# catid/longhair

Hardware: AMD Instinct MI355X
Metric: GB/s of input data encoded+decoded, device-resident, per GPU and whole node (higher is better)
Workload: dtype u8

## Files before the change

longhair_amd/csrc/codec.cpp:

```cpp
#include <hip/hip_runtime.h>

#include <algorithm>
#include <atomic>
#include <cstdio>
#include <cstdlib>
#include <cstring>
#include <map>
#include <memory>
#include <mutex>
#include <stdexcept>
#include <thread>
#include <string>
#include <vector>

#include "../../include/cauchy_256.h"
#include "../../include/cauchy_256_batch.h"
#include "field.hpp"
#include "jit.hpp"
#include "host_codec.hpp"
#include "kernels.hpp"

namespace lh {

enum { kOk = 0, kInvalid = -1, kNoDevice = -2, kHipError = -3 };
// ... 444 lines not shown
                        stride * (cfg.spw ? cfg.spw : 1) < (1ll << 31);
    const JitKernels *jk = nullptr;
    std::string err;
    if (jit_ok) {
        bool hard = false;
        jk = jit_lookup(d, cfg, allow_compile, &err, &hard);
        if (hard) return fail(kHipError, err);
    }
    JitConfig fcfg;
    if (!jk && k > 1 && m > 1 && !cfg.family && jit_family_config_for(k, m, bytes, &fcfg, true) &&
        stride * fcfg.spw < (1ll << 31)) {
        std::string ferr;
        bool fhard = false;
        if (const JitKernels *fk = jit_lookup(d, fcfg, allow_compile, &ferr, &fhard)) {
            if (fk->decode_fused) {
                jk = fk;
                cfg = fcfg;
            }
        }
    }
    const bool generic = (k > 1 && m > 1) && !jk;
    if (jk && jk->decode_fused && std::getenv("LONGHAIR_AMD_NO_FUSED_PLAN") == nullptr) {
        const uint8_t *zero = nullptr;
        if (int rc = zero_page(d, (size_t)bytes, &zero, st)) return rc;
        hipFunction_t fn = jk->decode_fused;
        long long s1 = stride;
        const uint8_t *gexp = d->gf_exp;
        const int16_t *glog = d->gf_log;
        int n = stripes, bb = bytes;
        void *args[] = {(void *)&d_blocks, &s1, (void *)&d_rows, (void *)&d_status, (void *)&zero,
                        (void *)&gexp, (void *)&glog, &n, &bb};
        const long long waves = cfg.spw ? (stripes + cfg.spw - 1) / cfg.spw : (long long)stripes * cfg.wps;
        const int wpb = cfg.family ? 4 : cfg.dec_wpb;
        LH_HIP(hipModuleLaunchKernel(fn, (unsigned)((waves + wpb - 1) / wpb), 1, 1, 64u * (unsigned)wpb, 1, 1,
                                     jk->dyn_lds, st, args, nullptr));
        note_launch(cfg.family ? "lh_jit_decode_fused(family)" : "lh_jit_decode_fused");
        return kOk;
    }
    JitConfig wcfg;
    const JitKernels *wk = nullptr;
    if (generic && jit_win_config_for(k, m, bytes, &wcfg, true)) {
        bool hard = false;
        wk = jit_lookup(d, wcfg, allow_compile, &err, &hard);
        if (hard) return fail(kHipError, err);
        if (wk && !wk->decode_wide) wk = nullptr;
    }
    const int sub = bytes / 8, jnch = (sub + 3) / 4;
    const bool jump = generic && !wk && sub >= 4 && !(sub % 4 != 0 && jnch > 1 && (jnch - 1) % 64 == 0);
    const size_t work_bytes = (generic && !wk && !jump) ? (size_t)stripes * e_max * bytes : 0;
    Workspace *w = nullptr;
    if (int rc = run_planner(d, st, k, m, e_max, stripes, d_rows, d_status, work_bytes, generic && !wk, &w)) return rc;
    if (k <= 1) return kOk;

    if (m == 1) {
        XorArgs a{};
        a.in = d_blocks;
        a.in_stride = stride;
        a.out = d_blocks;
        a.out_stride = stride;
        a.plan = w->plan.ptr;
        a.plan_stride = plan_stride;
        a.k = k;
        a.m = m;
        a.e_max = e_max;
        a.n_in = k;
        a.n_rep = 1;
        a.bytes = bytes;
        a.stripes = stripes;
// ... 1040 lines not shown
```

longhair_amd/csrc/jit.cpp:

```cpp
#include "jit.hpp"

#include <hip/hiprtc.h>
#include <dlfcn.h>
#include <sys/stat.h>
#include <unistd.h>
#include <utime.h>

#include <algorithm>
#include <cstdio>
#include <cstdlib>
#include <cstring>
#include <deque>
#include <functional>
#include <sstream>
#include <thread>

#include "field.hpp"

extern "C" const char lh_jit_source[];
extern "C" const char lh_inv_jump_source[];

namespace lh {

namespace {
// ... 67 lines not shown
    cfg->bytes = bytes;
    cfg->sub = sub;
    cfg->W = W;
    cfg->nch = nch2;
    cfg->spw = spw;
    cfg->wps = wps;
    cfg->lds = 0;
    if (W == 8 && nch2 <= 64 && bytes % 16 == 0) {
        bool dpp_ok = true;
        if (sub - 8 * (nch2 - 1) != 8)
            for (int s = 0; s < spw; ++s) dpp_ok = dpp_ok && (s * nch2 + nch2 - 1) % 16 != 0;
        cfg->lds = dpp_ok ? 1 : 0;
        const long long lq = ((long long)spw * bytes + 1023) / 1024;
        if (!decode && 4 * (4 * lq * 1024 + 16) + 4ll * spw * (k + m) * 8 > 80 * 1024) cfg->lds = 0;
    }
    cfg->role = decode ? 2 : 1;
    cfg->plain = decode && !(emax <= 4 && nch2 <= 64 && k <= 64 && std::getenv("LONGHAIR_AMD_NO_FUSED_PLAN") == nullptr);
    cfg->defines.clear();
    if (const char *d = std::getenv("LONGHAIR_AMD_JIT_DEFINES")) cfg->defines = d;
    auto knob = [&](const char *name, int dflt) {
        const size_t at = cfg->defines.find(name);
        return at == std::string::npos ? dflt : std::atoi(cfg->defines.c_str() + at + std::strlen(name));
    };
    const bool dmo = decode && cfg->lds && !cfg->plain && knob("LH_DMO=", 0) == 1;
    cfg->cps = 1;
    if ((!decode || dmo) && cfg->lds) cfg->cps = std::max(1, std::min(5, k / 2));
    cfg->cps = knob("LH_CPS=", cfg->cps);
    if (cfg->cps > 1 && !((!decode || dmo) && cfg->lds && k >= 2 * cfg->cps)) cfg->cps = 1;
    cfg->wgcu = knob("LH_WGCU=", cfg->cps > 1 ? 1 : 0);
    const int wpb = knob("LH_WPB=", 4);
    cfg->enc_wpb = (cfg->cps > 1 && wpb >= 1 && wpb <= 8) ? wpb : 4;
    const int dwpb = knob("LH_DWPB=", 4);
    cfg->dec_wpb = (decode && !cfg->plain && dwpb >= 1 && dwpb <= 8) ? dwpb : 4;
    cfg->family = 0;
    if (allow_family && knob("LH_FAMILY=", 0) && jit_family_config_for(k, m, bytes, cfg, decode)) return true;
    return true;
}

bool jit_family_config_for(int k, int m, int bytes, JitConfig *cfg, bool decode) {
    if (const char *env = std::getenv("LONGHAIR_AMD_PATH")) {
        if (std::string(env) == "generic") return false;
    }
    if (!jit_family_ok(k, m, bytes, decode)) return false;
    if (decode && std::getenv("LONGHAIR_AMD_NO_FUSED_PLAN") != nullptr) return false;
    JitConfig c;
    c.k = k;
    c.m = m;
    c.bytes = bytes;
    c.sub = bytes / 8;
    c.W = 8;
    c.nch = (c.sub + 7) / 8;
    c.spw = 64 / c.nch;
    c.wps = 0;
    c.lds = 1;
    c.role = decode ? 2 : 1;
    c.plain = 0;
    c.family = 1;
    if (const char *d = std::getenv("LONGHAIR_AMD_JIT_DEFINES")) c.defines = d;
    auto knob = [&](const char *name, int dflt) {
        const size_t at = c.defines.find(name);
        return at == std::string::npos ? dflt : std::atoi(c.defines.c_str() + at + std::strlen(name));
    };
    c.cps = std::max(2, std::min(5, k / 2));
    if (knob("LH_LDS=", 1) == 0 || knob("LH_CPS=", c.cps) < 2 || knob("LH_WPB=", 4) != 4) return false;
    c.wgcu = knob("LH_WGCU=", decode ? 0 : 1);
    c.enc_wpb = 4;
    *cfg = c;
    return true;
}

bool jit_ptr_config_for(int k, int m, int bytes, bool decode, JitConfig *cfg) {
    if (!config_impl(k, m, bytes, decode, cfg, false)) return false;
    cfg->cps = 1;
    cfg->enc_wpb = 4;
    if (cfg->defines.find("LH_WGCU=") == std::string::npos) cfg->wgcu = 0;
    if ((long long)(cfg->spw ? cfg->spw : 1) * k > 1024) return false;
    cfg->ptr = 1;
    const long long spw = cfg->spw ? cfg->spw : 1;
    if (decode && 4 * spw * (k + 1) * 8 > 4096) cfg->lds = 0;
    return true;
}

bool jit_win_ptr_config_for(int k, int m, int bytes, JitConfig *cfg, bool decode) {
    if (!jit_win_config_for(k, m, bytes, cfg, decode)) return false;
    cfg->ptr = 1;
    return true;
}

bool jit_win_config_for(int k, int m, int bytes, JitConfig *cfg, bool decode) {
    if (const char *env = std::getenv("LONGHAIR_AMD_PATH")) {
        if (std::string(env) == "generic") return false;
    }
    if (k < 2 || m < 2 || k + m > 256 || bytes % 8 != 0 || bytes <= 0) return false;
    const int sub = bytes / 8, W = 4;
    if (sub % (64 * W) != 0) return false;
    cfg->k = k;
    cfg->m = m;
    cfg->bytes = bytes;
    cfg->sub = sub;
// ... 281 lines not shown
       << "  const int p = (int)(blockIdx.x % lh_cps) * " << 64 * c.W << " + (int)(threadIdx.x & 63) * "
       << c.W << ";\n"
       << "  const unsigned char *b = in + stripe * in_stride + p;\n"
       << "  unsigned char *o = out + stripe * out_stride + p;\n";
    os << "  const unsigned char *sb = in + stripe * in_stride + (int)(blockIdx.x % lh_cps) * " << 64 * c.W
       << ";\n";
    const char *eargs = "(b, o, sb, nullptr, bytes, lh_sub)";
    for (int g = 0; g < NG; ++g) os << "  " << (g ? "else " : "") << "if (g == " << g << ") lh_wg" << g << eargs << ";\n";
    os << "}\n";
    return os.str();
}

std::string jit_source_for(const JitConfig &c) {
    std::ostringstream os;
    if (c.win) {
        std::string tok;
        for (char ch : c.defines + " ") {
            if (ch == ' ' || ch == ',') {
                const size_t eq = tok.find('=');
                if (!tok.empty()) os << "#define " << (eq == std::string::npos ? tok : tok.substr(0, eq) + " " + tok.substr(eq + 1)) << "\n";
                tok.clear();
            } else {
                tok += ch;
            }
        }
        os << win_source_for(c);
        return os.str();
    }
    {
        std::string tok;
        for (char ch : c.defines + " ") {
            if (ch == ' ' || ch == ',') {
                const size_t eq = tok.find('=');
                if (!tok.empty()) os << "#define " << (eq == std::string::npos ? tok : tok.substr(0, eq) + " " + tok.substr(eq + 1)) << "\n";
                tok.clear();
            } else {
                tok += ch;
            }
        }
    }
    if (c.family) {
        os << "#define LH_FAMILY 1\n#define LH_K " << c.k << "\n#define LH_M " << c.m
           << "\n#define LH_BYTES 1024\n#define LH_SUB 128\n#define LH_W 8\n#define LH_NCH 16\n#define LH_SPW 4"
              "\n#define LH_WPS 1\n#ifndef LH_LDS\n#define LH_LDS 1\n#endif\n#ifndef LH_CPS\n#define LH_CPS "
           << c.cps << "\n#endif\n#define LH_ROLE " << c.role << "\n#define LH_DEC_PLAIN 0\n";
    } else {
    os << "#define LH_K " << c.k << "\n#define LH_M " << c.m << "\n#define LH_BYTES " << c.bytes
       << "\n#define LH_SUB " << c.sub << "\n#define LH_W " << c.W << "\n#define LH_NCH " << c.nch
       << "\n#define LH_SPW " << (c.spw ? c.spw : 1) << "\n#define LH_WPS " << (c.wps ? c.wps : 1) << "\n";
    if (c.ptr) os << "#define LH_PTR 1\n#define LH_BUF 0\n";
    if (c.lds) os << "#ifndef LH_LDS\n#define LH_LDS 1\n#endif\n";
    if (c.cps > 1 && !c.ptr) os << "#ifndef LH_CPS\n#define LH_CPS " << c.cps << "\n#endif\n";
    if (c.role) os << "#define LH_ROLE " << c.role << "\n#define LH_DEC_PLAIN " << c.plain << "\n";
    }
    const std::vector<uint8_t> g = generator_matrix(c.k, c.m);
    os << "static constexpr unsigned char LH_BM[" << c.m << "][" << c.k << "][8] = {";
    for (int r = 0; r < c.m; ++r) {
        os << "{";
        for (int x = 0; x < c.k; ++x) {
            const uint64_t bm = bitmatrix(g[(size_t)r * c.k + x]);
            os << "{";
            for (int y = 0; y < 8; ++y) os << (unsigned)((bm >> (8 * y)) & 0xFF) << (y < 7 ? "," : "");
            os << "}" << (x + 1 < c.k ? "," : "");
        }
        os << "}" << (r + 1 < c.m ? "," : "");
    }
    os << "};\n";
// ... 364 lines not shown
```

longhair_amd/csrc/jit.hpp:

```cpp
#pragma once

#include <hip/hip_runtime.h>

#include <condition_variable>
#include <cstdint>
#include <map>
#include <memory>
#include <mutex>
#include <string>
#include <tuple>
#include <vector>

namespace lh {

struct JitConfig {
    int k, m, bytes, sub;
    int W;
    int nch;
    int spw;
    int wps;
    std::string defines;
    int win = 0;
    int rows_per_wave = 8;
    int win_pf = 3;
    int win_lds = 1;
    int win_split = 1;
    int ptr = 0;
    int lds = 0;
    int role = 0;
    int plain = 0;
    int wgcu = 0;
    int cps = 1;
    int family = 0;
    int enc_wpb = 4;
    int dec_wpb = 4;
    int lanes_per_launch_unit() const { return 64; }
};

struct JitKernels {
    hipModule_t module = nullptr;
    hipFunction_t encode = nullptr;
    hipFunction_t decode = nullptr;
    hipFunction_t decode_fused = nullptr;
    hipFunction_t encode_win = nullptr;
    hipFunction_t decode_wide = nullptr;
    unsigned dyn_lds = 0;
    JitConfig cfg{};
};

bool jit_config_for(int k, int m, int bytes, bool decode, JitConfig *cfg);

bool jit_ptr_config_for(int k, int m, int bytes, bool decode, JitConfig *cfg);

bool jit_win_config_for(int k, int m, int bytes, JitConfig *cfg, bool decode = false);
bool jit_win_ptr_config_for(int k, int m, int bytes, JitConfig *cfg, bool decode = false);

long long generator_ones(int k, int m);

bool jit_family_ok(int k, int m, int bytes, bool decode = false);
bool jit_family_config_for(int k, int m, int bytes, JitConfig *cfg, bool decode = false);

enum class JitMode {
    kCached,
    kAsync,
    kBlocking,
};

class JitCache {
// ... 36 lines not shown
```

longhair_amd/csrc/jit_codec.hip:

```cpp

#ifndef LH_K
#define LH_K 4
#define LH_M 2
#define LH_BYTES 64
#define LH_SUB 8
#define LH_W 8
#define LH_NCH 1
#define LH_SPW 64
#define LH_WPS 0
static constexpr unsigned char LH_BM[LH_M][LH_K][8] = {
    {{1, 2, 4, 8, 16, 32, 64, 128}, {1, 2, 4, 8, 16, 32, 64, 128},
     {1, 2, 4, 8, 16, 32, 64, 128}, {1, 2, 4, 8, 16, 32, 64, 128}},
    {{1, 2, 4, 8, 16, 32, 64, 128}, {2, 4, 8, 16, 32, 64, 128, 135},
     {3, 6, 12, 24, 48, 96, 192, 7}, {4, 8, 16, 32, 64, 128, 135, 137}}};
#define LH_G_INIT {{1, 1, 1, 1}, {1, 2, 3, 4}}
#include <hip/hip_runtime.h>
#endif

#define LH_NW ((LH_W + 3) / 4)


struct lh_word {
    unsigned int v[LH_NW];
};
// ... 1383 lines not shown
extern "C" __global__ void __launch_bounds__(256)
lh_jit_decode(unsigned char *__restrict__ blocks, long long stripe_stride,
              const unsigned char *__restrict__ plan, long long plan_stride,
              const unsigned char *__restrict__ zero_page, int stripes) {
    LH_WAVE_LOOP(stripes) { lh_decode_wave(lh_w, blocks, stripe_stride, plan, plan_stride, zero_page, stripes); }
}
#endif

#if LH_EMAX <= 4 && LH_NCH <= 64 && LH_K <= 64
#define LH_FUSED 1
#ifndef LH_DWPB
#define LH_DWPB 4
#endif
static constexpr unsigned char LH_GRAW[LH_M][LH_K] = LH_G_INIT;
#define LH_P4(n) (((n) + 3) / 4 * 4)
#define LH_SR (2 * LH_P4(LH_K) + LH_P4(LH_M))
#define LH_NRW ((LH_K + LH_NCH - 1) / LH_NCH)
#define LH_STRIPE_LANES (LH_NCH >= 64 ? ~0ull : ((1ull << (LH_NCH & 63)) - 1))

struct lh_gct {
    static constexpr int nch = LH_NCH, nrw = LH_NRW, maxrw = LH_NRW;
    static constexpr unsigned long long lanes = LH_STRIPE_LANES;
};

template <class G>
__device__ __forceinline__ void lh_fused_rows(const G &g, const lh_lane &l, int c, const unsigned char *__restrict__ rows,
                                              unsigned int (&rowv)[G::maxrw]) {
    const unsigned char *grow = rows + l.stripe * LH_K;
#pragma unroll
    for (int t = 0; t < G::maxrw; ++t) {
        const int i = c + t * g.nch;
        rowv[t] = (l.active && t < g.nrw && i < LH_K) ? (unsigned int)grow[i] : 0u;
    }
}

__device__ __forceinline__ unsigned int lh_gmul(const unsigned char *gexp, const short *glog, unsigned int a,
                                                unsigned int b) {
    return (a && b) ? gexp[glog[a] + glog[b]] : 0u;
}

struct lh_fused_solve {
    unsigned int rs[LH_EMAX], rr[LH_EMAX], er[LH_EMAX];
    unsigned char *grow;
    const unsigned char *gexp;
    const short *glog;
    const unsigned char *gmat;
    int c;
    __device__ __forceinline__ void operator()(lh_plan_regs &pr) const;
};

template <class G>
__device__ __forceinline__ bool lh_fused_plan(const G &g, const lh_lane &l, int c, int sl, unsigned char *scr,
                                              const unsigned int (&rowv)[G::maxrw],
                                              unsigned char *__restrict__ rows, signed char *__restrict__ status,
                                              lh_fused_solve &sv, lh_plan_regs &pr) {
    unsigned char *lrows = scr;
    unsigned char *lsrc = scr + LH_P4(LH_K);
    unsigned char *lrec = lsrc + LH_P4(LH_K);
    unsigned char *grow = rows + l.stripe * LH_K;
    for (int q = c; q < (LH_P4(LH_K) + LH_P4(LH_M)) / 4; q += g.nch) ((unsigned int *)lsrc)[q] = 0xFFFFFFFFu;
    bool bad = false;
#pragma unroll
    for (int t = 0; t < G::maxrw; ++t) {
        const int i = c + t * g.nch;
        if (t >= g.nrw || i >= LH_K) continue;
        const unsigned int r = rowv[t];
// ... 367 lines not shown
            }
#endif
#pragma unroll
            for (int y = 0; y < 8; ++y) {
                lh_word w = o[y];
                if constexpr (VL != 8) {
                    const lh_word f = lh_funnel<VL>(lh_row_shr1(w.v[0]), lh_row_shr1(w.v[1]), w.v[0], w.v[1]);
                    w.v[0] = last ? f.v[0] : w.v[0];
                    w.v[1] = last ? f.v[1] : w.v[1];
                }
#if LH_DEC_ST_PEND
                if (y == 7) {
                    pend = w;
                    pd = d;
                    continue;
                }
#endif
                lh_store(d + y * sub, w);
                asm volatile("" ::: "memory");
            }
        }
    }
#if LH_DEC_ST_PEND
    if (e > 0) lh_store(pd + 7 * sub, pend);
#endif
}
template <class DST>
__device__ __forceinline__ void lh_fused_out(const lh_word (&v)[LH_M][8], const lh_plan_regs &pr, bool last, DST dst) {
    lh_fused_out_g<LH_VLAST>(v, pr, last, LH_SUB, dst);
}
__device__ __forceinline__ void lh_fused_wave_lds(const lh_lane &l, long long wave, int c, int sl, bool work,
                                                  const unsigned char *scr, unsigned char *__restrict__ blocks,
                                                  long long stripe_stride, int stripes, const lh_fused_solve &sv,
                                                  lh_plan_regs &pr, const unsigned char *zero_page) {
    __shared__ __attribute__((aligned(16))) unsigned char lh_dring[LH_DWPB][LH_LD * LH_LQ * 1024 + LH_LPAD];
    const int lane = threadIdx.x & 63;
    const long long s0 = (long long)__builtin_amdgcn_readfirstlane((int)wave) * LH_SPW;
    if (s0 >= stripes) return;
    const int nst = (int)((stripes - s0) < LH_SPW ? (stripes - s0) : LH_SPW);
    const unsigned long long wm = __ballot(work);
    if (wm == 0) return;
    lh_dldsrc S;
#if LH_PTR
    __shared__ unsigned long long lh_dpt[LH_DWPB][LH_SPW * (LH_K + 1)];
    unsigned long long *prow = lh_dpt[threadIdx.x >> 6];
    __builtin_amdgcn_fence(__ATOMIC_RELEASE, "wavefront");
    __builtin_amdgcn_wave_barrier();
    if (sl < nst) {
        const unsigned long long *t = (const unsigned long long *)(blocks + (s0 + sl) * stripe_stride);
        for (int x = c; x <= LH_K; x += LH_NCH)
            prow[sl * (LH_K + 1) + x] = x < LH_K ? t[x] : (unsigned long long)zero_page;
    }
    __builtin_amdgcn_fence(__ATOMIC_RELEASE, "wavefront");
    __builtin_amdgcn_wave_barrier();
    __builtin_amdgcn_fence(__ATOMIC_ACQUIRE, "wavefront");
    S.pt = prow;
#else
    (void)zero_page;
#if LH_ASM_DMA
    S.rs = lh_rsrc(blocks + s0 * stripe_stride, (unsigned)(nst * stripe_stride));
#else
    S.rs = __builtin_amdgcn_make_buffer_rsrc(blocks + s0 * stripe_stride, 0, (int)(nst * stripe_stride), 0x00020000);
#endif
#endif
    S.scr = scr;
    S.ring = lh_dring[lh_wid<1>()];
#pragma unroll
    for (int q = 0; q < LH_LQ; ++q) {
        int j = 64 * q + lane;
        if (j >= nst * (LH_BYTES / 16)) j = nst * (LH_BYTES / 16) - 1;
        const int js = j / (LH_BYTES / 16);
#if LH_PTR
        S.prow[q] = js * (LH_K + 1);
        S.joff[q] = (j - js * (LH_BYTES / 16)) * 16;
#else
        S.joff[q] = js * (int)stripe_stride + (j - js * (LH_BYTES / 16)) * 16;
#endif
        S.jsc[q] = js * LH_SR | (((wm >> (js * LH_NCH)) & 1ull) ? 0 : (int)0x80000000);
    }
    asm volatile("s_waitcnt lgkmcnt(0)" ::: "memory");
    lh_decode_lds_prologue(S);
    if (work) sv(pr);
    lh_word v[LH_M][8];
#pragma unroll
    for (int r = 0; r < LH_M; ++r)
#pragma unroll
        for (int y = 0; y < 8; ++y)
#pragma unroll
            for (int i = 0; i < LH_NW; ++i) v[r][y].v[i] = 0;
    const int lo = (sl < LH_SPW ? sl : LH_SPW - 1) * LH_BYTES + 8 * c;
    int lo8 = lo + 8;
    asm volatile("" : "+v"(lo8));
    lh_unroll_decode_lds<0>::run(v, S, lo, lo8);
    if (!work) return;
#if LH_PTR
    lh_fused_out(v, pr, l.last, [&](int slot) {
        return (unsigned char *)S.pt[sl * (LH_K + 1) + slot] + (l.last ? LH_SUB - 8 : 8 * c);
    });
#else
    unsigned char *base = blocks + l.stripe * stripe_stride + (l.last ? LH_SUB - 8 : 8 * c);
    lh_fused_out(v, pr, l.last, [&](int slot) { return base + (long long)slot * LH_BYTES; });
#endif
}
#endif

#ifndef LH_DMO
#define LH_DMO 0
#endif
#if LH_DMO && !(LH_LDS && LH_CPS > 1 && !LH_PTR && defined(LH_FUSED))
#undef LH_DMO
#define LH_DMO 0
#endif
#if LH_DMO
#ifndef LH_DMO_AHEAD
// ... 51 lines not shown
        constexpr int S = (B * LH_SUB) % 8;
        if constexpr (S == 0) {
            d[B].v[0] = x[B].x;
            d[B].v[1] = x[B].y;
        } else {
            d[B] = lh_funnel<S>(x[B].x, x[B].y, y[B].x, y[B].y);
        }
        lh_dmo_fn<B + 1>(d, x, y);
    }
}
__device__ __forceinline__ void lh_dmo_col(lh_word (&d)[8], const unsigned char *col, int lo, int lo8) {
    lh_u32x2a x[8], y[8];
    lh_dmo_rd<0>(x, y, col, lo, lo8);
#pragma unroll
    for (int b = 0; b < 8; ++b) {
        asm volatile("" : "+v"(x[b]));
        if ((b * LH_SUB) % 8 != 0) asm volatile("" : "+v"(y[b]));
    }
    lh_dmo_fn<0>(d, x, y);
}
__device__ __forceinline__ void lh_dmo_issue(const lh_u32x4r &rs, const int (&voff)[LH_SQ], int t, unsigned char *ring) {
    const int lane = threadIdx.x & 63;
    const bool lastep = t + 1 == LH_NSTEP;
#pragma unroll
    for (int q = 0; q < LH_SQ; ++q) {
        int v = voff[q];
        if (LH_LASTC < LH_CPS && lastep) v = ((64 * q + lane) % LH_SCH) < LH_LASTC * LH_CCH ? v : (int)0x80000000;
        lh_dma16_bufs<LH_LDS_NT_DEC>(rs, v, t * (LH_CPS * LH_BYTES), ring + q * 1024);
    }
}
__device__ __forceinline__ void lh_fused_wave_dmo(const lh_lane &l, long long wave, int c, int sl, bool work,
                                                  const unsigned char *scr, unsigned char *__restrict__ blocks,
                                                  long long stripe_stride, int stripes, const lh_fused_solve &sv,
                                                  lh_plan_regs &pr) {
    __shared__ __attribute__((aligned(16))) unsigned char lh_mring[LH_DWPB][(1 + LH_DMO_AHEAD) * LH_SSLOT];
    const int lane = threadIdx.x & 63;
    const long long s0 = (long long)__builtin_amdgcn_readfirstlane((int)wave) * LH_SPW;
    if (s0 >= stripes) return;
    const int nst = (int)((stripes - s0) < LH_SPW ? (stripes - s0) : LH_SPW);
    const unsigned long long wm = __ballot(work);
    if (wm == 0) return;
    unsigned char *ring = lh_mring[lh_wid<1>()];
    const lh_u32x4r rs = lh_rsrc(blocks + s0 * stripe_stride, (unsigned)(nst * stripe_stride));
    int voff[LH_SQ];
#pragma unroll
    for (int q = 0; q < LH_SQ; ++q) {
        const int j = 64 * q + lane, js = j / LH_SCH, r = j - js * LH_SCH;
        const bool on = js < nst && ((wm >> (js * LH_NCH)) & 1ull);
        voff[q] = on ? js * (int)stripe_stride + r * 16 : (int)0x80000000;
    }
    asm volatile("s_waitcnt lgkmcnt(0)" ::: "memory");
    lh_dmo_issue(rs, voff, 0, ring);
    if (work) sv(pr);
    lh_word v[LH_M][8];
#pragma unroll
    for (int r = 0; r < LH_M; ++r)
#pragma unroll
        for (int y = 0; y < 8; ++y)
#pragma unroll
            for (int i = 0; i < LH_NW; ++i) v[r][y].v[i] = 0;
    const int sc = sl < LH_SPW ? sl : LH_SPW - 1;
    const int lo = sc * (LH_CPS * LH_BYTES) + 8 * c;
    int lo8 = lo + 8;
    asm volatile("" : "+v"(lo8));
    const unsigned char *lrows = scr + sc * LH_SR;
#pragma unroll 1
    for (int t = 0; t < LH_NSTEP; ++t) {
#if LH_DMO_AHEAD
        unsigned char *cur = ring + (t & 1) * LH_SSLOT;
        if (t + 1 < LH_NSTEP) {
            lh_dmo_issue(rs, voff, t + 1, ring + ((t + 1) & 1) * LH_SSLOT);
            lh_wait_vmcnt<LH_SQ>();
        } else {
            lh_wait_vmcnt<0>();
        }
#else
        unsigned char *cur = ring;
        lh_wait_vmcnt<0>();
#endif
        asm volatile("" ::: "memory");
        const int ncol = t + 1 < LH_NSTEP ? LH_CPS : LH_LASTC;
#pragma unroll 1
        for (int cc = 0; cc < ncol; ++cc) {
            lh_word d[8];
            lh_dmo_col(d, cur + cc * LH_BYTES, lo, lo8);
// ... 8 lines not shown
                const unsigned r = (unsigned)__builtin_amdgcn_readlane((int)row, (int)__builtin_ctzll(rem));
                unsigned diff = row ^ r;
                asm volatile("" : "+v"(diff));
                const bool mine = diff == 0u;
                rem &= ~__ballot(mine);
                if (mine) lh_rowdisp<0>::run(r, v, d);
            }
            lh_dopaque(v);
        }
        asm volatile("s_waitcnt lgkmcnt(0)" ::: "memory");
#if !LH_DMO_AHEAD
        if (t + 1 < LH_NSTEP) lh_dmo_issue(rs, voff, t + 1, ring);
#endif
    }
    if (!work) return;
    unsigned char *base = blocks + l.stripe * stripe_stride + (l.last ? LH_SUB - 8 : 8 * c);
    lh_fused_out(v, pr, l.last, [&](int slot) { return base + (long long)slot * LH_BYTES; });
}
#endif

#ifndef LH_DEC_LB
#define LH_DEC_LB 1
#endif
template <int PF>
__device__ __forceinline__ void lh_fused_body(unsigned char *__restrict__ blocks, long long stripe_stride,
                                              unsigned char *__restrict__ rows, signed char *__restrict__ status,
                                              const unsigned char *__restrict__ zero_page,
                                              const unsigned char *__restrict__ gf_exp,
                                              const short *__restrict__ gf_log, int stripes) {
    __shared__ unsigned char gexp[1024];
    __shared__ short glog[256];
    __shared__ unsigned char gmat[LH_M * LH_K];
    __shared__ __attribute__((aligned(16))) unsigned char scratch[LH_DWPB][LH_SPW > 0 ? LH_SPW : 1][LH_SR];
    for (int i = threadIdx.x; i < 256; i += blockDim.x) {
#pragma unroll
        for (int q = 0; q < 4; ++q) gexp[i + 256 * q] = gf_exp[(i + 256 * q) % 255];
        glog[i] = gf_log[i];
    }
    for (int i = threadIdx.x; i < LH_M * LH_K; i += blockDim.x) gmat[i] = LH_GRAW[i / LH_K][i % LH_K];
    __syncthreads();
    const int wid = threadIdx.x >> 6;
    LH_WAVE_LOOP(stripes) {
        const lh_lane l = lh_map_lane(stripes, lh_w);
        const int lane = threadIdx.x & 63;
        const int sl = lane / LH_NCH;
        const int c = lane - sl * LH_NCH;
        lh_plan_regs pr;
        lh_fused_solve sv;
        sv.gexp = gexp;
        sv.glog = glog;
        sv.gmat = gmat;
        unsigned int rowv[lh_gct::maxrw];
        lh_fused_rows(lh_gct(), l, c, rows, rowv);
#if LH_DMO
        const bool work = l.active && lh_fused_plan(lh_gct(), l, c, sl, &scratch[wid][sl][0], rowv, rows, status, sv, pr);
        lh_fused_wave_dmo(l, lh_w, c, sl, work, &scratch[wid][0][0], blocks, stripe_stride, stripes, sv, pr);
#elif LH_LDS
        const bool work = l.active && lh_fused_plan(lh_gct(), l, c, sl, &scratch[wid][sl][0], rowv, rows, status, sv, pr);
        lh_fused_wave_lds(l, lh_w, c, sl, work, &scratch[wid][0][0], blocks, stripe_stride, stripes, sv, pr, zero_page);
#else
        if (l.active && lh_fused_plan(lh_gct(), l, c, sl, &scratch[wid][sl][0], rowv, rows, status, sv, pr))
            lh_decode_body<PF>(l, lh_w, blocks, stripe_stride, pr, zero_page, stripes, sv);
#endif
    }
}

#if (LH_ROLE == 0 || (LH_ROLE == 2 && !LH_DEC_PLAIN)) && !LH_FAMILY
extern "C" __global__ void __launch_bounds__(64 * LH_DWPB, LH_DEC_LB)
lh_jit_decode_fused(unsigned char *__restrict__ blocks, long long stripe_stride, unsigned char *__restrict__ rows,
                    signed char *__restrict__ status, const unsigned char *__restrict__ zero_page,
                    const unsigned char *__restrict__ gf_exp, const short *__restrict__ gf_log, int stripes) {
    lh_fused_body<LH_PF_DEC>(blocks, stripe_stride, rows, status, zero_page, gf_exp, gf_log, stripes);
}
#endif

#if LH_FAMILY && LH_ROLE == 2 && LH_LDS && !LH_PTR
#define LH_FNRW 8
#define LH_FSPW (64 / ((LH_K + LH_FNRW - 1) / LH_FNRW))
#define LH_FRS (4 * 1024 + 16)
struct lh_grt {
    int nch, nrw;
    unsigned long long lanes;
    static constexpr int maxrw = LH_FNRW;
};
struct lh_dfam {
    int bytes, sub, nch, spw, cch;
};
struct lh_fdsrc {
    __amdgpu_buffer_rsrc_t rs;
    int joff[4], jsc[4];
    int bytes;
    const unsigned char *scr;
    unsigned char *ring;
    template <int X>
    __device__ __forceinline__ void slots(unsigned (&sv)[4]) const {
#pragma unroll
        for (int q = 0; q < 4; ++q) {
            const unsigned b = scr[(jsc[q] & 0x7FFFFFFF) + lh_dmoff<X>::v];
            sv[q] = jsc[q] < 0 ? 0xFFu : b;
        }
    }
    __device__ __forceinline__ void issue(const unsigned (&sv)[4], int slot) const {
#pragma unroll
        for (int q = 0; q < 4; ++q) {
            int off = slot * LH_FRS + q * 1024;
            asm volatile("" : "+s"(off));
            __builtin_amdgcn_raw_ptr_buffer_load_lds(
                rs, (__attribute__((address_space(3))) void *)(ring + off), 16,
                sv[q] == 0xFFu ? (int)0x80000000 : joff[q] + (int)sv[q] * bytes, 0, 0, LH_LDS_NT_DEC ? 2 : 0);
        }
    }
};
template <int C, int N>
__device__ __forceinline__ void lh_fdslots(const lh_fdsrc &S, unsigned (&sv)[LH_LDG][4]) {
    if constexpr (N > 0 && C < LH_DCOLS) {
        S.slots<C>(sv[LH_LDG - N]);
        lh_fdslots<C + 1, N - 1>(S, sv);
    }
}
template <int C, int N>
// ... 38 lines not shown
            asm volatile("" ::: "memory");
            lh_word d[8];
#if LH_DFAM_PIN
            lh_fam_col<R>(d, S.ring + (X % LH_LD) * LH_FRS, ad, ad8);
#else
            lh_dfam_col<R>(d, S.ring + (X % LH_LD) * LH_FRS, ad);
#endif
            lh_dcombine<X, LH_LDS_REC_FIRST>(v, d);
            lh_dopaque(v);
            if constexpr (LH_LDG == 1 && X + LH_LD < LH_DCOLS) {
                asm volatile("s_waitcnt lgkmcnt(0)" ::: "memory");
                S.issue(sv, X % LH_LD);
            } else if constexpr (refill) {
                asm volatile("s_waitcnt lgkmcnt(0)" ::: "memory");
                lh_fdissue<LH_LD + X + 1 - LH_LDG, LH_LDG>(S, svg);
            }
            lh_unroll_dfam<X + 1, R>::run(v, S, ad, ad8);
        }
    }
};
template <int X = 0>
__device__ __forceinline__ void lh_dfam_prologue(const lh_fdsrc &S) {
    if constexpr (X < LH_LD && X < LH_DCOLS) {
        unsigned sv[4];
        S.slots<X>(sv);
        S.issue(sv, X);
        lh_dfam_prologue<X + 1>(S);
    }
}
template <int R>
__device__ __forceinline__ void lh_fused_wave_fam(const lh_dfam &F, const lh_lane &l, long long wave, int c, int sl, bool work,
                                                  const unsigned char *scr, unsigned char *__restrict__ blocks,
                                                  long long stripe_stride, int stripes, const lh_fused_solve &sv,
                                                  lh_plan_regs &pr, unsigned char *ring) {
    const int lane = threadIdx.x & 63;
    const long long s0 = (long long)__builtin_amdgcn_readfirstlane((int)wave) * F.spw;
    if (s0 >= stripes) return;
    const int nst = (int)((stripes - s0) < F.spw ? (stripes - s0) : F.spw);
    const unsigned long long wm = __ballot(work);
    if (wm == 0) return;
    lh_fdsrc S;
    S.rs = __builtin_amdgcn_make_buffer_rsrc(blocks + s0 * stripe_stride, 0, (int)(nst * stripe_stride), 0x00020000);
    S.bytes = F.bytes;
    S.scr = scr;
    S.ring = ring;
#pragma unroll
    for (int q = 0; q < 4; ++q) {
        const int j = 64 * q + lane;
        const int js = j / F.cch;
        const bool on = js < nst && ((wm >> (js * F.nch)) & 1ull);
        S.joff[q] = js * (int)stripe_stride + (j - js * F.cch) * 16;
        S.jsc[q] = on ? js * LH_SR : (int)0x80000000;
    }
    asm volatile("s_waitcnt lgkmcnt(0)" ::: "memory");
    lh_dfam_prologue(S);
    if (work) sv(pr);
    lh_word v[LH_M][8];
#pragma unroll
    for (int r = 0; r < LH_M; ++r)
#pragma unroll
        for (int y = 0; y < 8; ++y)
#pragma unroll
            for (int i = 0; i < LH_NW; ++i) v[r][y].v[i] = 0;
    const int lo = (sl < F.spw ? sl : F.spw - 1) * F.bytes + 8 * c;
    int ad[8], ad8[8];
#pragma unroll
    for (int b = 0; b < 8; ++b) {
        ad[b] = lo + b * (F.sub - R);
        ad8[b] = ad[b] + 8;
#if LH_FAM_SPLIT
        asm volatile("" : "+v"(ad8[b]));
#endif
    }
    lh_unroll_dfam<0, R>::run(v, S, ad, ad8);
    if (!work) return;
    unsigned char *base = blocks + l.stripe * stripe_stride + (l.last ? F.sub - 8 : 8 * c);
    lh_fused_out_g<R == 0 ? 8 : R>(v, pr, l.last, F.sub, [&](int slot) { return base + (long long)slot * F.bytes; });
}
template <int R>
__device__ __forceinline__ void lh_dfam_body(const lh_dfam &F, const lh_grt &g, unsigned char *__restrict__ blocks,
                                             long long stripe_stride, unsigned char *__restrict__ rows,
                                             signed char *__restrict__ status, const unsigned char *gexp, const short *glog,
                                             const unsigned char *gmat, unsigned char (*scratch)[LH_FSPW][LH_SR],
                                             unsigned char *ring, int stripes) {
    const int wid = threadIdx.x >> 6, lane = threadIdx.x & 63;
    const int sl = lane / F.nch, c = lane - sl * F.nch;
    const long long nw = ((long long)stripes + F.spw - 1) / F.spw;
    const long long ws = (long long)gridDim.x * (blockDim.x >> 6);
    for (long long w = (lh_block_id() * blockDim.x + threadIdx.x) >> 6; w < nw; w += ws) {
        lh_lane l;
        l.stripe = w * F.spw + sl;
        l.active = sl < F.spw && l.stripe < stripes;
        l.last = c == F.nch - 1;
        l.p = 0;
        lh_plan_regs pr;
        lh_fused_solve sv;
        sv.gexp = gexp;
        sv.glog = glog;
        sv.gmat = gmat;
        unsigned int rowv[LH_FNRW];
        lh_fused_rows(g, l, c, rows, rowv);
        const bool work = l.active && lh_fused_plan(g, l, c, sl, &scratch[wid][sl][0], rowv, rows, status, sv, pr);
        lh_fused_wave_fam<R>(F, l, w, c, sl, work, &scratch[wid][0][0], blocks, stripe_stride, stripes, sv, pr, ring);
    }
}
extern "C" __global__ void __launch_bounds__(256, LH_DEC_LB)
lh_jit_decode_fused(unsigned char *__restrict__ blocks, long long stripe_stride, unsigned char *__restrict__ rows,
                    signed char *__restrict__ status, const unsigned char *__restrict__ zero_page,
                    const unsigned char *__restrict__ gf_exp, const short *__restrict__ gf_log, int stripes, int bytes) {
    (void)zero_page;
    __shared__ unsigned char gexp[1024];
    __shared__ short glog[256];
    __shared__ unsigned char gmat[LH_M * LH_K];
    __shared__ __attribute__((aligned(16))) unsigned char scratch[4][LH_FSPW][LH_SR];
    __shared__ __attribute__((aligned(16))) unsigned char lh_fdring[4][LH_LD * LH_FRS];
    for (int i = threadIdx.x; i < 256; i += blockDim.x) {
#pragma unroll
        for (int q = 0; q < 4; ++q) gexp[i + 256 * q] = gf_exp[(i + 256 * q) % 255];
        glog[i] = gf_log[i];
    }
    for (int i = threadIdx.x; i < LH_M * LH_K; i += blockDim.x) gmat[i] = LH_GRAW[i / LH_K][i % LH_K];
    __syncthreads();
    lh_dfam F;
    F.bytes = bytes;
    F.sub = bytes >> 3;
    F.nch = (F.sub + 7) >> 3;
    F.spw = 64 / F.nch;
    F.cch = bytes >> 4;
    lh_grt g;
    g.nch = F.nch;
    g.nrw = (LH_K + F.nch - 1) / F.nch;
    g.lanes = F.nch >= 64 ? ~0ull : ((1ull << F.nch) - 1);
    unsigned char *ring = lh_fdring[__builtin_amdgcn_readfirstlane((int)(threadIdx.x >> 6))];
    switch (F.sub & 7) {
        case 0: lh_dfam_body<0>(F, g, blocks, stripe_stride, rows, status, gexp, glog, gmat, scratch, ring, stripes); break;
        case 2: lh_dfam_body<2>(F, g, blocks, stripe_stride, rows, status, gexp, glog, gmat, scratch, ring, stripes); break;
        case 4: lh_dfam_body<4>(F, g, blocks, stripe_stride, rows, status, gexp, glog, gmat, scratch, ring, stripes); break;
        default: lh_dfam_body<6>(F, g, blocks, stripe_stride, rows, status, gexp, glog, gmat, scratch, ring, stripes); break;
    }
}
#endif

#endif
```

Measured before the change: 4770.

## Overlap fused-decode table setup and row loads with first stripe's work

Fused decode kernels no longer fill the GF exp/log and matrix tables in LDS and then barrier before any work starts. Each wave now issues its first row loads and the table loads into registers up front, writes the tables to LDS, and defers the block barrier until just before the solve needs the tables. The next iteration's rows are prefetched at the end of each loop pass. A new LH_DGRID knob can also cap the decode grid size so the launch becomes persistent-style; it defaults off. This hides global-load latency at kernel start, at the cost of more registers and more complex barrier handling.

```diff
diff --git a/longhair_amd/csrc/codec.cpp b/longhair_amd/csrc/codec.cpp
--- a/longhair_amd/csrc/codec.cpp
+++ b/longhair_amd/csrc/codec.cpp
@@ -500,8 +500,10 @@
                         (void *)&gexp, (void *)&glog, &n, &bb};
         const long long waves = cfg.spw ? (stripes + cfg.spw - 1) / cfg.spw : (long long)stripes * cfg.wps;
         const int wpb = cfg.family ? 4 : cfg.dec_wpb;
-        LH_HIP(hipModuleLaunchKernel(fn, (unsigned)((waves + wpb - 1) / wpb), 1, 1, 64u * (unsigned)wpb, 1, 1,
-                                     jk->dyn_lds, st, args, nullptr));
+        long long grid = (waves + wpb - 1) / wpb;
+        if (cfg.dgrid > 0 && grid > cfg.dgrid) grid = cfg.dgrid;
+        LH_HIP(hipModuleLaunchKernel(fn, (unsigned)grid, 1, 1, 64u * (unsigned)wpb, 1, 1, jk->dyn_lds, st, args,
+                                     nullptr));
         note_launch(cfg.family ? "lh_jit_decode_fused(family)" : "lh_jit_decode_fused");
         return kOk;
     }
diff --git a/longhair_amd/csrc/jit.cpp b/longhair_amd/csrc/jit.cpp
--- a/longhair_amd/csrc/jit.cpp
+++ b/longhair_amd/csrc/jit.cpp
@@ -123,6 +123,7 @@
     cfg->enc_wpb = (cfg->cps > 1 && wpb >= 1 && wpb <= 8) ? wpb : 4;
     const int dwpb = knob("LH_DWPB=", 4);
     cfg->dec_wpb = (decode && !cfg->plain && dwpb >= 1 && dwpb <= 8) ? dwpb : 4;
+    cfg->dgrid = decode ? std::max(0, knob("LH_DGRID=", 0)) : 0;
     cfg->family = 0;
     if (allow_family && knob("LH_FAMILY=", 0) && jit_family_config_for(k, m, bytes, cfg, decode)) return true;
     return true;
@@ -156,6 +157,7 @@
     if (knob("LH_LDS=", 1) == 0 || knob("LH_CPS=", c.cps) < 2 || knob("LH_WPB=", 4) != 4) return false;
     c.wgcu = knob("LH_WGCU=", decode ? 0 : 1);
     c.enc_wpb = 4;
+    c.dgrid = decode ? std::max(0, knob("LH_DGRID=", 0)) : 0;
     *cfg = c;
     return true;
 }
@@ -503,7 +505,8 @@
         for (char ch : c.defines + " ") {
             if (ch == ' ' || ch == ',') {
                 const size_t eq = tok.find('=');
-                if (!tok.empty()) os << "#define " << (eq == std::string::npos ? tok : tok.substr(0, eq) + " " + tok.substr(eq + 1)) << "\n";
+                if (!tok.empty() && tok.compare(0, 9, "LH_DGRID=") != 0)
+                    os << "#define " << (eq == std::string::npos ? tok : tok.substr(0, eq) + " " + tok.substr(eq + 1)) << "\n";
                 tok.clear();
             } else {
                 tok += ch;
diff --git a/longhair_amd/csrc/jit.hpp b/longhair_amd/csrc/jit.hpp
--- a/longhair_amd/csrc/jit.hpp
+++ b/longhair_amd/csrc/jit.hpp
@@ -34,6 +34,7 @@
     int family = 0;
     int enc_wpb = 4;
     int dec_wpb = 4;
+    int dgrid = 0;
     int lanes_per_launch_unit() const { return 64; }
 };
 
diff --git a/longhair_amd/csrc/jit_codec.hip b/longhair_amd/csrc/jit_codec.hip
--- a/longhair_amd/csrc/jit_codec.hip
+++ b/longhair_amd/csrc/jit_codec.hip
@@ -1439,6 +1439,54 @@
         const int i = c + t * g.nch;
         rowv[t] = (l.active && t < g.nrw && i < LH_K) ? (unsigned int)grow[i] : 0u;
     }
+}
+
+template <int NT>
+struct lh_fused_tables {
+    static constexpr int NE = (256 + NT - 1) / NT, NG = (LH_M * LH_K + NT - 1) / NT;
+    unsigned int ex[NE][4], lg[NE], gm[NG];
+    __device__ __forceinline__ void load(const unsigned char *__restrict__ gf_exp, const short *__restrict__ gf_log) {
+#pragma unroll
+        for (int t = 0; t < NE; ++t) {
+            const int i = (int)threadIdx.x + t * NT < 256 ? (int)threadIdx.x + t * NT : 255;
+#pragma unroll
+            for (int q = 0; q < 4; ++q) ex[t][q] = gf_exp[(i + 256 * q) % 255];
+            lg[t] = (unsigned int)(unsigned short)gf_log[i];
+        }
+#pragma unroll
+        for (int t = 0; t < NG; ++t) {
+            const int i = (int)threadIdx.x + t * NT < LH_M * LH_K ? (int)threadIdx.x + t * NT : LH_M * LH_K - 1;
+            gm[t] = LH_GRAW[i / LH_K][i % LH_K];
+        }
+    }
+    __device__ __forceinline__ void store(unsigned char *gexp, short *glog, unsigned char *gmat) const {
+#pragma unroll
+        for (int t = 0; t < NE; ++t) {
+            const int i = (int)threadIdx.x + t * NT;
+            if (i < 256) {
+#pragma unroll
+                for (int q = 0; q < 4; ++q) gexp[i + 256 * q] = (unsigned char)ex[t][q];
+                glog[i] = (short)lg[t];
+            }
+        }
+#pragma unroll
+        for (int t = 0; t < NG; ++t) {
+            const int i = (int)threadIdx.x + t * NT;
+            if (i < LH_M * LH_K) gmat[i] = (unsigned char)gm[t];
+        }
+    }
+};
+__device__ __forceinline__ void lh_fused_sync(int &pend) {
+    if (__builtin_amdgcn_readfirstlane(pend)) {
+        asm volatile("s_waitcnt lgkmcnt(0)\n\ts_barrier" ::: "memory");
+        pend = 0;
+    }
+}
+
+template <int N>
+__device__ __forceinline__ void lh_rows_landed(unsigned int (&rowv)[N]) {
+#pragma unroll
+    for (int t = 0; t < N; ++t) asm volatile("" : "+v"(rowv[t]));
 }
 
 __device__ __forceinline__ unsigned int lh_gmul(const unsigned char *gexp, const short *glog, unsigned int a,
@@ -1872,7 +1920,7 @@
 __device__ __forceinline__ void lh_fused_wave_lds(const lh_lane &l, long long wave, int c, int sl, bool work,
                                                   const unsigned char *scr, unsigned char *__restrict__ blocks,
                                                   long long stripe_stride, int stripes, const lh_fused_solve &sv,
-                                                  lh_plan_regs &pr, const unsigned char *zero_page) {
+                                                  lh_plan_regs &pr, const unsigned char *zero_page, int &pend) {
     __shared__ __attribute__((aligned(16))) unsigned char lh_dring[LH_DWPB][LH_LD * LH_LQ * 1024 + LH_LPAD];
     const int lane = threadIdx.x & 63;
     const long long s0 = (long long)__builtin_amdgcn_readfirstlane((int)wave) * LH_SPW;
@@ -1920,6 +1968,7 @@
     }
     asm volatile("s_waitcnt lgkmcnt(0)" ::: "memory");
     lh_decode_lds_prologue(S);
+    lh_fused_sync(pend);
     if (work) sv(pr);
     lh_word v[LH_M][8];
 #pragma unroll
@@ -2037,7 +2086,7 @@
 __device__ __forceinline__ void lh_fused_wave_dmo(const lh_lane &l, long long wave, int c, int sl, bool work,
                                                   const unsigned char *scr, unsigned char *__restrict__ blocks,
                                                   long long stripe_stride, int stripes, const lh_fused_solve &sv,
-                                                  lh_plan_regs &pr) {
+                                                  lh_plan_regs &pr, int &pend) {
     __shared__ __attribute__((aligned(16))) unsigned char lh_mring[LH_DWPB][(1 + LH_DMO_AHEAD) * LH_SSLOT];
     const int lane = threadIdx.x & 63;
     const long long s0 = (long long)__builtin_amdgcn_readfirstlane((int)wave) * LH_SPW;
@@ -2056,6 +2105,7 @@
     }
     asm volatile("s_waitcnt lgkmcnt(0)" ::: "memory");
     lh_dmo_issue(rs, voff, 0, ring);
+    lh_fused_sync(pend);
     if (work) sv(pr);
     lh_word v[LH_M][8];
 #pragma unroll
@@ -2130,37 +2180,44 @@
     __shared__ short glog[256];
     __shared__ unsigned char gmat[LH_M * LH_K];
     __shared__ __attribute__((aligned(16))) unsigned char scratch[LH_DWPB][LH_SPW > 0 ? LH_SPW : 1][LH_SR];
-    for (int i = threadIdx.x; i < 256; i += blockDim.x) {
-#pragma unroll
-        for (int q = 0; q < 4; ++q) gexp[i + 256 * q] = gf_exp[(i + 256 * q) % 255];
-        glog[i] = gf_log[i];
-    }
-    for (int i = threadIdx.x; i < LH_M * LH_K; i += blockDim.x) gmat[i] = LH_GRAW[i / LH_K][i % LH_K];
-    __syncthreads();
     const int wid = threadIdx.x >> 6;
-    LH_WAVE_LOOP(stripes) {
-        const lh_lane l = lh_map_lane(stripes, lh_w);
-        const int lane = threadIdx.x & 63;
-        const int sl = lane / LH_NCH;
-        const int c = lane - sl * LH_NCH;
+    const int lane = threadIdx.x & 63;
+    const int sl = lane / LH_NCH;
+    const int c = lane - sl * LH_NCH;
+    const long long nw = lh_total_waves(stripes);
+    const long long ws = (long long)gridDim.x * LH_DWPB;
+    long long w = (lh_block_id() * (64 * LH_DWPB) + threadIdx.x) >> 6;
+    lh_lane l = lh_map_lane(stripes, w);
+    unsigned int rowv[lh_gct::maxrw];
+    lh_fused_rows(lh_gct(), l, c, rows, rowv);
+    {
+        lh_fused_tables<64 * LH_DWPB> tb;
+        tb.load(gf_exp, gf_log);
+        tb.store(gexp, glog, gmat);
+    }
+    int pend = 1;
+    for (; w < nw; w += ws) {
+        lh_rows_landed(rowv);
         lh_plan_regs pr;
         lh_fused_solve sv;
         sv.gexp = gexp;
         sv.glog = glog;
         sv.gmat = gmat;
-        unsigned int rowv[lh_gct::maxrw];
-        lh_fused_rows(lh_gct(), l, c, rows, rowv);
 #if LH_DMO
         const bool work = l.active && lh_fused_plan(lh_gct(), l, c, sl, &scratch[wid][sl][0], rowv, rows, status, sv, pr);
-        lh_fused_wave_dmo(l, lh_w, c, sl, work, &scratch[wid][0][0], blocks, stripe_stride, stripes, sv, pr);
+        lh_fused_wave_dmo(l, w, c, sl, work, &scratch[wid][0][0], blocks, stripe_stride, stripes, sv, pr, pend);
 #elif LH_LDS
         const bool work = l.active && lh_fused_plan(lh_gct(), l, c, sl, &scratch[wid][sl][0], rowv, rows, status, sv, pr);
-        lh_fused_wave_lds(l, lh_w, c, sl, work, &scratch[wid][0][0], blocks, stripe_stride, stripes, sv, pr, zero_page);
-#else
-        if (l.active && lh_fused_plan(lh_gct(), l, c, sl, &scratch[wid][sl][0], rowv, rows, status, sv, pr))
-            lh_decode_body<PF>(l, lh_w, blocks, stripe_stride, pr, zero_page, stripes, sv);
-#endif
-    }
+        lh_fused_wave_lds(l, w, c, sl, work, &scratch[wid][0][0], blocks, stripe_stride, stripes, sv, pr, zero_page, pend);
+#else
+        const bool work = l.active && lh_fused_plan(lh_gct(), l, c, sl, &scratch[wid][sl][0], rowv, rows, status, sv, pr);
+        lh_fused_sync(pend);
+        if (work) lh_decode_body<PF>(l, w, blocks, stripe_stride, pr, zero_page, stripes, sv);
+#endif
+        l = lh_map_lane(stripes, w + ws);
+        lh_fused_rows(lh_gct(), l, c, rows, rowv);
+    }
+    lh_fused_sync(pend);
 }
 
 #if (LH_ROLE == 0 || (LH_ROLE == 2 && !LH_DEC_PLAIN)) && !LH_FAMILY
@@ -2184,6 +2241,14 @@
 struct lh_dfam {
     int bytes, sub, nch, spw, cch;
 };
+__device__ __forceinline__ lh_lane lh_dfam_lane(const lh_dfam &F, int stripes, long long w, int sl, int c) {
+    lh_lane l;
+    l.stripe = w * F.spw + sl;
+    l.active = sl < F.spw && l.stripe < stripes;
+    l.last = c == F.nch - 1;
+    l.p = 0;
+    return l;
+}
 struct lh_fdsrc {
     __amdgpu_buffer_rsrc_t rs;
     int joff[4], jsc[4];
@@ -2288,7 +2353,7 @@
 __device__ __forceinline__ void lh_fused_wave_fam(const lh_dfam &F, const lh_lane &l, long long wave, int c, int sl, bool work,
                                                   const unsigned char *scr, unsigned char *__restrict__ blocks,
                                                   long long stripe_stride, int stripes, const lh_fused_solve &sv,
-                                                  lh_plan_regs &pr, unsigned char *ring) {
+                                                  lh_plan_regs &pr, unsigned char *ring, int &pend) {
     const int lane = threadIdx.x & 63;
     const long long s0 = (long long)__builtin_amdgcn_readfirstlane((int)wave) * F.spw;
     if (s0 >= stripes) return;
@@ -2310,6 +2375,7 @@
     }
     asm volatile("s_waitcnt lgkmcnt(0)" ::: "memory");
     lh_dfam_prologue(S);
+    lh_fused_sync(pend);
     if (work) sv(pr);
     lh_word v[LH_M][8];
 #pragma unroll
@@ -2338,26 +2404,23 @@
                                              long long stripe_stride, unsigned char *__restrict__ rows,
                                              signed char *__restrict__ status, const unsigned char *gexp, const short *glog,
                                              const unsigned char *gmat, unsigned char (*scratch)[LH_FSPW][LH_SR],
-                                             unsigned char *ring, int stripes) {
+                                             unsigned char *ring, int stripes, long long w, lh_lane l,
+                                             unsigned int (&rowv)[LH_FNRW], int &pend) {
     const int wid = threadIdx.x >> 6, lane = threadIdx.x & 63;
     const int sl = lane / F.nch, c = lane - sl * F.nch;
     const long long nw = ((long long)stripes + F.spw - 1) / F.spw;
     const long long ws = (long long)gridDim.x * (blockDim.x >> 6);
-    for (long long w = (lh_block_id() * blockDim.x + threadIdx.x) >> 6; w < nw; w += ws) {
-        lh_lane l;
-        l.stripe = w * F.spw + sl;
-        l.active = sl < F.spw && l.stripe < stripes;
-        l.last = c == F.nch - 1;
-        l.p = 0;
+    for (; w < nw; w += ws) {
+        lh_rows_landed(rowv);
         lh_plan_regs pr;
         lh_fused_solve sv;
         sv.gexp = gexp;
         sv.glog = glog;
         sv.gmat = gmat;
-        unsigned int rowv[LH_FNRW];
+        const bool work = l.active && lh_fused_plan(g, l, c, sl, &scratch[wid][sl][0], rowv, rows, status, sv, pr);
+        lh_fused_wave_fam<R>(F, l, w, c, sl, work, &scratch[wid][0][0], blocks, stripe_stride, stripes, sv, pr, ring, pend);
+        l = lh_dfam_lane(F, stripes, w + ws, sl, c);
         lh_fused_rows(g, l, c, rows, rowv);
-        const bool work = l.active && lh_fused_plan(g, l, c, sl, &scratch[wid][sl][0], rowv, rows, status, sv, pr);
-        lh_fused_wave_fam<R>(F, l, w, c, sl, work, &scratch[wid][0][0], blocks, stripe_stride, stripes, sv, pr, ring);
     }
 }
 extern "C" __global__ void __launch_bounds__(256, LH_DEC_LB)
@@ -2370,13 +2433,6 @@
     __shared__ unsigned char gmat[LH_M * LH_K];
     __shared__ __attribute__((aligned(16))) unsigned char scratch[4][LH_FSPW][LH_SR];
     __shared__ __attribute__((aligned(16))) unsigned char lh_fdring[4][LH_LD * LH_FRS];
-    for (int i = threadIdx.x; i < 256; i += blockDim.x) {
-#pragma unroll
-        for (int q = 0; q < 4; ++q) gexp[i + 256 * q] = gf_exp[(i + 256 * q) % 255];
-        glog[i] = gf_log[i];
-    }
-    for (int i = threadIdx.x; i < LH_M * LH_K; i += blockDim.x) gmat[i] = LH_GRAW[i / LH_K][i % LH_K];
-    __syncthreads();
     lh_dfam F;
     F.bytes = bytes;
     F.sub = bytes >> 3;
@@ -2387,14 +2443,27 @@
     g.nch = F.nch;
     g.nrw = (LH_K + F.nch - 1) / F.nch;
     g.lanes = F.nch >= 64 ? ~0ull : ((1ull << F.nch) - 1);
+    const int lane = threadIdx.x & 63;
+    const int sl = lane / F.nch, c = lane - sl * F.nch;
+    const long long w = (lh_block_id() * blockDim.x + threadIdx.x) >> 6;
+    const lh_lane l = lh_dfam_lane(F, stripes, w, sl, c);
+    unsigned int rowv[LH_FNRW];
+    lh_fused_rows(g, l, c, rows, rowv);
+    {
+        lh_fused_tables<256> tb;
+        tb.load(gf_exp, gf_log);
+        tb.store(gexp, glog, gmat);
+    }
+    int pend = 1;
     unsigned char *ring = lh_fdring[__builtin_amdgcn_readfirstlane((int)(threadIdx.x >> 6))];
     switch (F.sub & 7) {
-        case 0: lh_dfam_body<0>(F, g, blocks, stripe_stride, rows, status, gexp, glog, gmat, scratch, ring, stripes); break;
-        case 2: lh_dfam_body<2>(F, g, blocks, stripe_stride, rows, status, gexp, glog, gmat, scratch, ring, stripes); break;
-        case 4: lh_dfam_body<4>(F, g, blocks, stripe_stride, rows, status, gexp, glog, gmat, scratch, ring, stripes); break;
-        default: lh_dfam_body<6>(F, g, blocks, stripe_stride, rows, status, gexp, glog, gmat, scratch, ring, stripes); break;
-    }
-}
-#endif
-
-#endif
+        case 0: lh_dfam_body<0>(F, g, blocks, stripe_stride, rows, status, gexp, glog, gmat, scratch, ring, stripes, w, l, rowv, pend); break;
+        case 2: lh_dfam_body<2>(F, g, blocks, stripe_stride, rows, status, gexp, glog, gmat, scratch, ring, stripes, w, l, rowv, pend); break;
+        case 4: lh_dfam_body<4>(F, g, blocks, stripe_stride, rows, status, gexp, glog, gmat, scratch, ring, stripes, w, l, rowv, pend); break;
+        default: lh_dfam_body<6>(F, g, blocks, stripe_stride, rows, status, gexp, glog, gmat, scratch, ring, stripes, w, l, rowv, pend); break;
+    }
+    lh_fused_sync(pend);
+}
+#endif
+
+#endif
```

Result: slower. 4644 (-2.6%).
